# Immortal-ibr/Verifiable-Federated-Training-with-Zero-Knowledge-Proofs-ZK-FL-

Measured on AMD Instinct MI355X. Metric: Groth16 proofs/sec (training-step circuit, ~2^18 constraints) at 1/8 MI355X, higher is better.
Workload: dtype u32; 1 GPU; groth16 prove, sgd_verified(128, 4, 7, 1000) (BATCH,DIM,DEPTH,PRECISION); constraints=261399, wires=262810, domain=262144, global_batch=20, step=20 proofs per GPU (one per slot), parallelism=replicas1, slots_in_flight=20, hw_queues=28

## Files before the change

include/zkfl.h:

```cpp
#ifndef ZKFL_H
#define ZKFL_H

#include <stddef.h>
#include <stdint.h>

#ifdef __cplusplus
extern "C" {
#endif

#define ZKFL_OK 0
#define ZKFL_E_ARG -1
#define ZKFL_E_FORMAT -2
#define ZKFL_E_PRIME -3
#define ZKFL_E_MISMATCH -4
#define ZKFL_E_DEVICE -5
#define ZKFL_E_OOM -6
#define ZKFL_E_CONSTRAINT -7
#define ZKFL_E_KEY -8

typedef struct zkfl_ctx zkfl_ctx;
typedef struct zkfl_key zkfl_key;
typedef struct zkfl_witness zkfl_witness;
typedef struct zkfl_wprog zkfl_wprog;
typedef struct zkfl_vkey zkfl_vkey;
// ... 66 lines not shown
int zkfl_witness_free(zkfl_witness* w);
int zkfl_groth16_prove_resident(zkfl_ctx* ctx, zkfl_key* key, const zkfl_witness* w, const uint8_t* rs,
                                uint8_t proof_out[256]);
int zkfl_groth16_prove_batch(zkfl_ctx* ctx, zkfl_key* key, size_t n, const zkfl_witness* const* w,
                             const uint8_t* rs, uint8_t* proofs_out);

int zkfl_groth16_prove_multi(zkfl_ctx* ctx, size_t n, zkfl_key* const* keys, const zkfl_witness* const* w,
                             const uint8_t* rs, uint8_t* proofs_out);

int zkfl_zkey_load_shard(zkfl_ctx* ctx, const uint8_t* buf, size_t len, uint32_t shard, uint32_t n_shards,
                         zkfl_key** out);
int zkfl_key_shard(const zkfl_key* key, uint32_t* shard, uint32_t* n_shards);
int zkfl_groth16_prove_part_batch(zkfl_ctx* ctx, zkfl_key* key, size_t n, const zkfl_witness* const* w,
                                  const uint8_t* rs, uint8_t* parts_out);
int zkfl_groth16_assemble(zkfl_ctx* ctx, size_t n, size_t n_parts, const uint8_t* parts, const uint8_t* rs,
                          uint8_t* proofs_out);

int zkfl_debug_prove_parts(zkfl_ctx* ctx, zkfl_key* key, const uint8_t* wtns, size_t wtns_len, uint8_t* h_out,
                           uint8_t* msm_out);

int zkfl_debug_glv_split(const uint8_t k[32], uint8_t out[40]);

int zkfl_debug_g1_glv_mul(zkfl_ctx* ctx, size_t n, const uint8_t* points, const uint8_t* scalars, uint8_t* out);

int zkfl_debug_msm_front(zkfl_ctx* ctx, uint32_t n1, const size_t* n, const uint8_t* const* bases,
                         const uint8_t* const* scalars, const size_t* n_scalars, const uint32_t* const* sidx,
                         const uint32_t* extra_start, const uint8_t* const* extra, const size_t* n_extra, uint32_t b,
                         const uint8_t* bases_g2, size_t n_b, int fast, int joint, uint8_t* out_g1, uint8_t out_g2[128]);

int zkfl_debug_wtrace(zkfl_ctx* ctx, int op, uint32_t cap, void* out, uint32_t* count);

int zkfl_debug_ntt_coset(zkfl_ctx* ctx, uint8_t* data, uint32_t logn, uint32_t nvec, size_t vstride, int col_max);

int zkfl_msm_g1(zkfl_ctx* ctx, const uint8_t* bases, const uint8_t* scalars, size_t n, uint8_t out[64]);
int zkfl_msm_g2(zkfl_ctx* ctx, const uint8_t* bases, const uint8_t* scalars, size_t n, uint8_t out[128]);
int zkfl_ntt_coset(zkfl_ctx* ctx, uint8_t* data, uint32_t logn);

int zkfl_wprog_load(zkfl_ctx* ctx, const uint8_t* prog, size_t len, zkfl_wprog** out);
int zkfl_wprog_free(zkfl_wprog* prog);
int zkfl_wprog_info(const zkfl_wprog* prog, uint32_t* n_wires, uint32_t* n_inputs, uint32_t* n_public);
size_t zkfl_wtns_size(const zkfl_wprog* prog);
int zkfl_wprog_parse_inputs(const uint8_t* prog, size_t len, const char* input_json, uint8_t* inputs_out, size_t cap,
                            size_t* n_inputs);
int zkfl_witness_compute_json(zkfl_ctx* ctx, const zkfl_wprog* prog, const char* input_json, uint8_t* wtns_out);
int zkfl_witness_compute(zkfl_ctx* ctx, const zkfl_wprog* prog, size_t n, const uint8_t* inputs, uint8_t* wtns_out);
int zkfl_witness_compute_resident(zkfl_ctx* ctx, const zkfl_wprog* prog, const zkfl_key* key, size_t n,
                                  const uint8_t* inputs, zkfl_witness** out);

int zkfl_groth16_full_prove_batch(zkfl_ctx* ctx, zkfl_key* key, const zkfl_wprog* prog, size_t n,
                                  const uint8_t* inputs, const uint8_t* rs, uint8_t* proofs_out, uint8_t* pubs_out);

int zkfl_groth16_full_prove_json(zkfl_ctx* ctx, zkfl_key* key, const zkfl_wprog* prog, const char* input_json,
                                 const uint8_t* rs, uint8_t proof_out[256], uint8_t* pub_out);

int zkfl_groth16_full_prove_json_batch(zkfl_ctx* ctx, zkfl_key* key, const zkfl_wprog* prog, size_t n,
                                       const char* const* input_jsons, const uint8_t* rs, uint8_t* proofs_out,
                                       uint8_t* pubs_out);

int zkfl_groth16_full_prove_multi(zkfl_ctx* ctx, size_t n, zkfl_key* const* keys, const zkfl_wprog* const* progs,
                                  const uint8_t* const* inputs, const uint8_t* rs, uint8_t* proofs_out,
                                  uint8_t* const* pubs_out);

typedef struct zkfl_r1cs zkfl_r1cs;
typedef struct {
  uint32_t n_wires, n_pub_out, n_pub_in, n_prv_in, n_constraints;
  uint64_t n_labels, n_terms;
// ... 136 lines not shown
```

verifiable-federated-training-with-zero-knowledge-proofs-zk-fl-_amd/csrc/field.h:

```cpp
#pragma once
#include <hip/hip_runtime.h>
#include <stdint.h>

namespace zkfl {

#define ZK_DEV __device__ __forceinline__

struct FqP {
  static constexpr uint32_t P[8] = {0xd87cfd47u, 0x3c208c16u, 0x6871ca8du, 0x97816a91u,
                                    0x8181585du, 0xb85045b6u, 0xe131a029u, 0x30644e72u};
  static constexpr uint32_t ONE[8] = {0xc58f0d9du, 0xd35d438du, 0xf5c70b3du, 0x0a78eb28u,
                                      0x7879462cu, 0x666ea36fu, 0x9a07df2fu, 0x0e0a77c1u};
  static constexpr uint32_t R2[8] = {0x538afa89u, 0xf32cfc5bu, 0xd44501fbu, 0xb5e71911u,
                                     0x0a417ff6u, 0x47ab1effu, 0xcab8351fu, 0x06d89f71u};
  static constexpr uint32_t INV = 0xe4866389u;
};

struct FrP {
  static constexpr uint32_t P[8] = {0xf0000001u, 0x43e1f593u, 0x79b97091u, 0x2833e848u,
                                    0x8181585du, 0xb85045b6u, 0xe131a029u, 0x30644e72u};
  static constexpr uint32_t ONE[8] = {0x4ffffffbu, 0xac96341cu, 0x9f60cd29u, 0x36fc7695u,
                                      0x7879462eu, 0x666ea36fu, 0x9a07df2fu, 0x0e0a77c1u};
  static constexpr uint32_t R2[8] = {0xae216da7u, 0x1bb8e645u, 0xe35c59e3u, 0x53fe3ab1u,
                                     0x53bb8085u, 0x8c49833du, 0x7f4e44a5u, 0x0216d0b1u};
  static constexpr uint32_t INV = 0xefffffffu;
};

template <class PR>
struct Fp {
  uint32_t v[8];
};

using Fq = Fp<FqP>;
using Fr = Fp<FrP>;

template <class PR>
ZK_DEV Fp<PR> fp_zero() {
  Fp<PR> r;
#pragma unroll
  for (int i = 0; i < 8; i++) r.v[i] = 0;
  return r;
}

template <class PR>
ZK_DEV Fp<PR> fp_one() {
  Fp<PR> r;
#pragma unroll
  for (int i = 0; i < 8; i++) r.v[i] = PR::ONE[i];
  return r;
}

template <class PR>
ZK_DEV bool fp_is_zero(const Fp<PR>& a) {
  uint32_t x = 0;
#pragma unroll
  for (int i = 0; i < 8; i++) x |= a.v[i];
  return x == 0;
}

template <class PR>
ZK_DEV bool fp_eq(const Fp<PR>& a, const Fp<PR>& b) {
  uint32_t x = 0;
#pragma unroll
  for (int i = 0; i < 8; i++) x |= a.v[i] ^ b.v[i];
  return x == 0;
}

template <class PR>
ZK_DEV void fp_reduce_once(uint32_t r[8], const uint32_t a[8]) {
  uint32_t t[8];
  uint32_t borrow = 0;
#pragma unroll
  for (int i = 0; i < 8; i++) {
    uint64_t d = (uint64_t)a[i] - PR::P[i] - borrow;
    t[i] = (uint32_t)d;
    borrow = (uint32_t)(d >> 63);
  }
#pragma unroll
  for (int i = 0; i < 8; i++) r[i] = borrow ? a[i] : t[i];
}

template <class PR>
ZK_DEV Fp<PR> fp_add(const Fp<PR>& a, const Fp<PR>& b) {
  uint32_t s[8];
  uint64_t c = 0;
#pragma unroll
  for (int i = 0; i < 8; i++) {
    c += (uint64_t)a.v[i] + b.v[i];
    s[i] = (uint32_t)c;
    c >>= 32;
  }
  Fp<PR> r;
  fp_reduce_once<PR>(r.v, s);
  return r;
}

template <class PR>
ZK_DEV Fp<PR> fp_sub(const Fp<PR>& a, const Fp<PR>& b) {
  uint32_t d[8];
  uint32_t borrow = 0;
#pragma unroll
  for (int i = 0; i < 8; i++) {
    uint64_t t = (uint64_t)a.v[i] - b.v[i] - borrow;
    d[i] = (uint32_t)t;
    borrow = (uint32_t)(t >> 63);
  }
  uint32_t mask = 0u - borrow;
  uint64_t c = 0;
  Fp<PR> r;
#pragma unroll
  for (int i = 0; i < 8; i++) {
    c += (uint64_t)d[i] + (PR::P[i] & mask);
    r.v[i] = (uint32_t)c;
    c >>= 32;
  }
  return r;
}

template <class PR>
ZK_DEV Fp<PR> fp_neg(const Fp<PR>& a) {
  return fp_sub<PR>(fp_zero<PR>(), a);
}

template <class PR>
ZK_DEV Fp<PR> fp_dbl(const Fp<PR>& a) {
  return fp_add<PR>(a, a);
}

#define ZK_MAC_VV(lo, hi, x, y)                                                                             \
  do {                                                                                                      \
    uint64_t cc_;                                                                                           \
    asm("v_mad_u64_u32 %0, %1, %3, %4, %0\n\tv_addc_co_u32 %2, %1, %2, 0, %1" : "+v"(lo), "=&s"(cc_), "+v"(hi) \
        : "v"(x), "v"(y));                                                                                  \
  } while (0)
#define ZK_MAC_VS(lo, hi, x, y)                                                                             \
  do {                                                                                                      \
    uint64_t cc_;                                                                                           \
    asm("v_mad_u64_u32 %0, %1, %3, %4, %0\n\tv_addc_co_u32 %2, %1, %2, 0, %1" : "+v"(lo), "=&s"(cc_), "+v"(hi) \
        : "v"(x), "s"(y));                                                                                  \
  } while (0)

template <class PR>
ZK_DEV Fp<PR> fp_mul(const Fp<PR>& a, const Fp<PR>& b) {
  uint32_t m[8], u[9];
  uint64_t lo = 0;
  uint32_t hi = 0;
#pragma unroll
  for (int i = 0; i < 8; i++) {
#pragma unroll
    for (int j = 0; j < i; j++) {
      ZK_MAC_VV(lo, hi, a.v[j], b.v[i - j]);
      ZK_MAC_VS(lo, hi, m[j], PR::P[i - j]);
    }
    ZK_MAC_VV(lo, hi, a.v[i], b.v[0]);
    m[i] = (uint32_t)lo * PR::INV;
    ZK_MAC_VS(lo, hi, m[i], PR::P[0]);
    lo = (lo >> 32) | ((uint64_t)hi << 32);
    hi = 0;
  }
#pragma unroll
  for (int i = 8; i < 16; i++) {
#pragma unroll
    for (int j = i - 7; j < 8; j++) {
      ZK_MAC_VV(lo, hi, a.v[j], b.v[i - j]);
      ZK_MAC_VS(lo, hi, m[j], PR::P[i - j]);
    }
    u[i - 8] = (uint32_t)lo;
    lo = (lo >> 32) | ((uint64_t)hi << 32);
    hi = 0;
  }
  u[8] = (uint32_t)lo;
  Fp<PR> r;
  fp_reduce_once<PR>(r.v, u);
  return r;
}

template <class PR>
ZK_DEV Fp<PR> fp_mul_sum2(const Fp<PR>& a, const Fp<PR>& b, const Fp<PR>& c, const Fp<PR>& d) {
  uint32_t m[8], u[9];
  uint64_t lo = 0;
  uint32_t hi = 0;
#pragma unroll
  for (int i = 0; i < 8; i++) {
#pragma unroll
    for (int j = 0; j < i; j++) {
      ZK_MAC_VV(lo, hi, a.v[j], b.v[i - j]);
      ZK_MAC_VV(lo, hi, c.v[j], d.v[i - j]);
      ZK_MAC_VS(lo, hi, m[j], PR::P[i - j]);
    }
    ZK_MAC_VV(lo, hi, a.v[i], b.v[0]);
    ZK_MAC_VV(lo, hi, c.v[i], d.v[0]);
    m[i] = (uint32_t)lo * PR::INV;
    ZK_MAC_VS(lo, hi, m[i], PR::P[0]);
    lo = (lo >> 32) | ((uint64_t)hi << 32);
    hi = 0;
  }
#pragma unroll
  for (int i = 8; i < 16; i++) {
#pragma unroll
    for (int j = i - 7; j < 8; j++) {
      ZK_MAC_VV(lo, hi, a.v[j], b.v[i - j]);
      ZK_MAC_VV(lo, hi, c.v[j], d.v[i - j]);
      ZK_MAC_VS(lo, hi, m[j], PR::P[i - j]);
    }
    u[i - 8] = (uint32_t)lo;
    lo = (lo >> 32) | ((uint64_t)hi << 32);
    hi = 0;
  }
  u[8] = (uint32_t)lo;
  Fp<PR> r;
  fp_reduce_once<PR>(r.v, u);
  return r;
}

template <class PR>
ZK_DEV Fp<PR> fp_sqr(const Fp<PR>& a) {
  return fp_mul<PR>(a, a);
}

template <class PR>
ZK_DEV Fp<PR> fp_to_mont(const Fp<PR>& a) {
  Fp<PR> r2;
#pragma unroll
  for (int i = 0; i < 8; i++) r2.v[i] = PR::R2[i];
  return fp_mul<PR>(a, r2);
}

template <class PR>
ZK_DEV Fp<PR> fp_from_mont(const Fp<PR>& a) {
  Fp<PR> one;
  one.v[0] = 1;
#pragma unroll
  for (int i = 1; i < 8; i++) one.v[i] = 0;
  return fp_mul<PR>(a, one);
}

template <class PR>
ZK_DEV Fp<PR> fp_pow(const Fp<PR>& a, const uint32_t e[8]) {
  Fp<PR> r = fp_one<PR>();
#pragma unroll
  for (int i = 7; i >= 0; i--) {
#pragma unroll 1
    for (int b = 31; b >= 0; b--) {
      r = fp_sqr<PR>(r);
      if ((e[i] >> b) & 1u) r = fp_mul<PR>(r, a);
    }
  }
  return r;
}

template <class PR>
ZK_DEV Fp<PR> fp_inv(const Fp<PR>& a) {
  uint32_t e[8];
  uint32_t borrow = 2;
#pragma unroll
  for (int i = 0; i < 8; i++) {
    uint64_t d = (uint64_t)PR::P[i] - borrow;
    e[i] = (uint32_t)d;
    borrow = (uint32_t)(d >> 63);
  }
  return fp_pow<PR>(a, e);
}
// ... 84 lines not shown
```

verifiable-federated-training-with-zero-knowledge-proofs-zk-fl-_amd/csrc/groups.hip:

```cpp
#include <hip/hip_runtime.h>
#include <stdint.h>

#include <chrono>
#include <cstdio>
#include <vector>

#include "devbufs.h"
#include "groups.h"
#include "objects.h"

using namespace zkfl;

namespace {

ZK_DEV Fq from_m29(const Fq& a) {
  Fq c = fp_zero<FqP>();
  c.v[7] = 0x08000000u;
  return fp_mul(a, c);
}

template <class F>
ZK_DEV Affine<F> load_base(const Affine<F>* __restrict__ p) {
  Affine<F> a = *p;
  Fq* q = reinterpret_cast<Fq*>(&a);
#pragma unroll
  for (int k = 0; k < (int)(sizeof(Affine<F>) / sizeof(Fq)); k++) q[k] = from_m29(q[k]);
  return a;
}

template <class F>
__global__ void __launch_bounds__(64) k_group_sums(const Affine<F>* __restrict__ bases_w, int W, size_t n,
                                                   const uint32_t* __restrict__ start,
                                                   const uint32_t* __restrict__ members, Affine<F>* __restrict__ out) {
  const size_t j = (size_t)blockIdx.x * blockDim.x + threadIdx.x;
  if (j >= n) return;
  const Affine<F> p = load_base<F>(bases_w + j * W);
  const uint32_t b = start[j], e = start[j + 1];
  if (b == e) {
    out[j] = p;
    return;
  }
  XYZZ<F> acc = xyzz_from_affine<F>(p);
  for (uint32_t m = b; m < e; m++) acc = xyzz_madd<F>(acc, load_base<F>(bases_w + (size_t)members[m] * W));
  out[j] = xyzz_to_affine<F>(acc);
}

constexpr int DELTA_T = 256;

__global__ void __launch_bounds__(DELTA_T) k_group_delta(const Fr* __restrict__ w, const uint32_t* __restrict__ rep,
                                                         uint32_t n, Fr* __restrict__ u, uint32_t* __restrict__ cnt,
                                                         uint32_t* __restrict__ miss_out, const GroupMark M) {
  ZK_LIGHT();
  const uint32_t i = blockIdx.x * DELTA_T + threadIdx.x;
  int nz = 0;
  if (i < n) {
    const uint32_t r = rep[i];
    Fr v = fp_zero<FrP>();
    if (r != i) {
      v = fp_sub(w[i], w[r]);
#pragma unroll
      for (int k = 0; k < 8; k++) nz |= v.v[k] != 0;
    }
    u[i] = v;
  }
  if (M.wstart) {
    const unsigned long long m = __ballot(nz);
    if (m) {
      const uint32_t lane = threadIdx.x & (warpSize - 1);
      const int first = __ffsll((long long)m) - 1;
      uint32_t base = 0;
      if ((int)lane == first) base = atomicAdd(&M.state[2], (uint32_t)__popcll(m));
      base = __shfl(base, first);
      const uint32_t at = base + (uint32_t)__popcll(m & ((1ull << lane) - 1ull));
      if (nz && at < M.miss_cap) M.missing[at] = i;
    }
  }
  const int blk = __syncthreads_count(nz);
  if (threadIdx.x == 0) {
    if (blk) atomicAdd(&cnt[0], (uint32_t)blk);
    __threadfence();
    if (atomicAdd(&cnt[1], 1u) == gridDim.x - 1) {
      __threadfence();
      miss_out[0] = atomicExch(&cnt[0], 0u);
      cnt[1] = 0;
    }
  }
}

constexpr int MARK_T = 256, MARK_BLOCKS_MAX = 256;

__global__ void __launch_bounds__(MARK_T) k_group_mark(const GroupMark M) {
  ZK_LIGHT();
  const uint32_t n = M.state[2];
  if (n == 0) return;
  if (n > M.miss_cap) {
    if (blockIdx.x == 0 && threadIdx.x == 0) atomicExch(&M.state[1], 1u);
    return;
  }
  const uint32_t lane = threadIdx.x & (warpSize - 1), per = MARK_T / warpSize;
  for (uint32_t k = blockIdx.x * per + threadIdx.x / warpSize; k < n; k += gridDim.x * per) {
    if (__any((int)__atomic_load_n(&M.state[1], __ATOMIC_RELAXED))) return;
    const uint32_t i = M.missing[k], s = M.wstart[i], e = M.wstart[i + 1] & ~GROUP_ROWS_OVER;
    if (s & GROUP_ROWS_OVER) {
      if (lane == 0) atomicExch(&M.state[1], 1u);
      return;
    }
    for (uint32_t p = s + lane; p < e; p += warpSize) {
      const uint32_t j = M.wlist[p], bit = 1u << (j & 31);
      if (atomicOr(&M.state[GROUP_ROWS_STATE_BITS + (j >> 5)], bit) & bit) continue;
      const uint32_t at = atomicAdd(&M.state[0], 1u);
      if (at < M.cap) M.dirty[at] = j;
      else atomicExch(&M.state[1], 1u);
    }
  }
}

}

namespace zkfl {

template <class F>
void group_sums(hipStream_t st, const Affine<F>* bases_w, int W, size_t n, const uint32_t* start,
                const uint32_t* members, Affine<F>* out) {
  if (n) hipLaunchKernelGGL(k_group_sums<F>, dim3(zk_grid(n, 64)), dim3(64), 0, st, bases_w, W, n, start, members, out);
}
template void group_sums<FqOps>(hipStream_t, const G1Aff*, int, size_t, const uint32_t*, const uint32_t*, G1Aff*);
template void group_sums<Fq2Ops>(hipStream_t, const G2Aff*, int, size_t, const uint32_t*, const uint32_t*, G2Aff*);

void group_delta(hipStream_t st, const Fr* w, const uint32_t* rep, uint32_t n, Fr* u, uint32_t* cnt,
                 uint32_t* miss_out, const GroupMark& mark) {
  hipLaunchKernelGGL(k_group_delta, dim3(zk_grid(n, DELTA_T)), dim3(DELTA_T), 0, st, w, rep, n, u, cnt, miss_out, mark);
}

void group_mark_rows(hipStream_t st, const GroupMark& mark) {
  const unsigned blocks = std::min<unsigned>(zk_grid((size_t)mark.miss_cap * 64, MARK_T), MARK_BLOCKS_MAX);
  hipLaunchKernelGGL(k_group_mark, dim3(blocks), dim3(MARK_T), 0, st, mark);
}

void key_groups_release(zkfl_key* k) {
  msm_bases_free(k->gA);
  msm_bases_free(k->gB1);
  msm_bases_free(k->gB2);
  msm_bases_free(k->gCH);
  void* ptrs[] = {k->grp.d_rep,    k->grp.d_cls,    k->grp.d_crp,  k->grp.d_cterms,
                  k->grp.d_ccoefs, k->grp.d_wstart, k->grp.d_wlist};
  for (void* p : ptrs)
    if (p) (void)hipFree(p);
  const uint32_t builds = k->grp.builds;
  k->grp = KeyGroups();
  k->grp.builds = builds;
}

}

namespace {

template <class F>
hipError_t build_query(const MsmBases<F>& plain, MsmBases<F>& out, const GroupQuery& q, uint32_t extra_start,
                       DevBufs& D, hipStream_t st) {
  ZK_CHECK(msm_bases_alloc(out, plain.n, plain.c));
  if (plain.n == 0) return hipSuccess;
  uint32_t *d_start, *d_members;
  Affine<F>* d_img;
  ZK_CHECK(D.get(&d_start, q.start.size()));
// ... 259 lines not shown
```

verifiable-federated-training-with-zero-knowledge-proofs-zk-fl-_amd/csrc/ntt.hip:

```cpp
#include "ntt.h"
#include "devbufs.h"
#include "fr_consts.h"
#include "wtrace.h"

namespace zkfl {

#ifndef NTT_LDS_LOG_BITS
#define NTT_LDS_LOG_BITS 10
#endif
constexpr int NTT_LDS_LOG = NTT_LDS_LOG_BITS;
constexpr int NTT_LDS_N = 1 << NTT_LDS_LOG;

__global__ void k_ntt_twiddles(Fr* __restrict__ tw, size_t half, Fr root_mont) {
  size_t i = (size_t)blockIdx.x * blockDim.x + threadIdx.x;
  if (i >= half) return;
  Fr acc = fp_one<FrP>();
  Fr base = root_mont;
  size_t e = i;
  while (e) {
    if (e & 1) acc = fp_mul(acc, base);
    base = fp_sqr(base);
    e >>= 1;
  }
  tw[i] = acc;
// ... 18 lines not shown
                                size_t twstride, int nvec, size_t vstride) {
  size_t t = (size_t)blockIdx.x * blockDim.x + threadIdx.x;
  size_t nb = n >> 1;
  if (t >= nb * nvec) return;
  size_t v = t / nb;
  t -= v * nb;
  Fr* x = a + v * vstride;
  size_t j = t & (half - 1);
  size_t i0 = ((t - j) << 1) + j;
  size_t i1 = i0 + half;
  Fr u = x[i0], w = x[i1];
  x[i0] = fp_add(u, w);
  x[i1] = fp_mul(fp_sub(u, w), tw[j * twstride]);
}

__global__ void k_ntt_dit_stage(Fr* __restrict__ a, size_t n, size_t half, const Fr* __restrict__ tw,
                                size_t twstride, int nvec, size_t vstride) {
  size_t t = (size_t)blockIdx.x * blockDim.x + threadIdx.x;
  size_t nb = n >> 1;
  if (t >= nb * nvec) return;
  size_t v = t / nb;
  t -= v * nb;
  Fr* x = a + v * vstride;
  size_t j = t & (half - 1);
  size_t i0 = ((t - j) << 1) + j;
  size_t i1 = i0 + half;
  Fr u = x[i0];
  Fr w = fp_mul(x[i1], tw[j * twstride]);
  x[i0] = fp_add(u, w);
  x[i1] = fp_sub(u, w);
}

template <bool DIF>
__global__ void __launch_bounds__(512) k_ntt_lds(Fr* __restrict__ a, size_t n, int logt,
                                                 const Fr* __restrict__ tw, int nvec, size_t vstride,
                                                 const Fr* __restrict__ scale) {
  __shared__ Fr tile[NTT_LDS_N];
  const size_t T = (size_t)1 << logt;
  const size_t tiles_per_vec = n >> logt;
  const size_t tile_id = blockIdx.x;
  const size_t v = tile_id / tiles_per_vec;
  if (v >= (size_t)nvec) return;
  Fr* x = a + v * vstride + (tile_id - v * tiles_per_vec) * T;
  for (size_t i = threadIdx.x; i < T; i += blockDim.x) tile[i] = x[i];
  __syncthreads();
  const size_t nbf = T >> 1;
  for (int s = 0; s < logt; s++) {
    const size_t half = DIF ? (T >> (s + 1)) : ((size_t)1 << s);
    const size_t len = half << 1;
    const size_t twstride = n / len;
    for (size_t t = threadIdx.x; t < nbf; t += blockDim.x) {
      size_t j = t & (half - 1);
      size_t i0 = ((t - j) << 1) + j;
      size_t i1 = i0 + half;
      Fr u = tile[i0], w = tile[i1];
      Fr tws = tw[j * twstride];
      if (DIF) {
        tile[i0] = fp_add(u, w);
        tile[i1] = fp_mul(fp_sub(u, w), tws);
      } else {
        w = fp_mul(w, tws);
        tile[i0] = fp_add(u, w);
        tile[i1] = fp_sub(u, w);
      }
    }
    __syncthreads();
  }
  const size_t base = (tile_id - v * tiles_per_vec) * T;
  if (scale)
    for (size_t i = threadIdx.x; i < T; i += blockDim.x) x[i] = fp_mul(tile[i], scale[base + i]);
  else
    for (size_t i = threadIdx.x; i < T; i += blockDim.x) x[i] = tile[i];
}

__global__ void __launch_bounds__(512) k_ntt_lds_pair(Fr* __restrict__ a, size_t n, int logt,
                                                      const Fr* __restrict__ tw_inv, const Fr* __restrict__ tw_fwd,
                                                      int nvec, size_t vstride, const Fr* __restrict__ scale) {
  ZK_WT(WT_NTT_LDS);
  ZK_LIGHT();
  __shared__ Fr tile[NTT_LDS_N];
  const size_t T = (size_t)1 << logt;
  const size_t tiles_per_vec = n >> logt;
  const size_t tile_id = blockIdx.x;
  const size_t v = tile_id / tiles_per_vec;
  if (v >= (size_t)nvec) return;
  const size_t base = (tile_id - v * tiles_per_vec) * T;
  Fr* x = a + v * vstride + base;
  for (size_t i = threadIdx.x; i < T; i += blockDim.x) tile[i] = x[i];
  __syncthreads();
  const size_t nbf = T >> 1;
  for (int s = 0; s < logt; s++) {
    const size_t half = T >> (s + 1), twstride = n / (half << 1);
    for (size_t t = threadIdx.x; t < nbf; t += blockDim.x) {
      const size_t j = t & (half - 1), i0 = ((t - j) << 1) + j, i1 = i0 + half;
      const Fr u = tile[i0], w = tile[i1];
      tile[i0] = fp_add(u, w);
      tile[i1] = fp_mul(fp_sub(u, w), tw_inv[j * twstride]);
    }
    __syncthreads();
  }
  for (size_t i = threadIdx.x; i < T; i += blockDim.x) tile[i] = fp_mul(tile[i], scale[base + i]);
  __syncthreads();
  for (int s = 0; s < logt; s++) {
    const size_t half = (size_t)1 << s, twstride = n / (half << 1);
    for (size_t t = threadIdx.x; t < nbf; t += blockDim.x) {
      const size_t j = t & (half - 1), i0 = ((t - j) << 1) + j, i1 = i0 + half;
      const Fr u = tile[i0], w = fp_mul(tile[i1], tw_fwd[j * twstride]);
      tile[i0] = fp_add(u, w);
      tile[i1] = fp_sub(u, w);
    }
    __syncthreads();
  }
  for (size_t i = threadIdx.x; i < T; i += blockDim.x) x[i] = tile[i];
}

template <bool DIF>
__global__ void __launch_bounds__(256) k_ntt_lds4(Fr* __restrict__ a, size_t n, int logt, const Fr* __restrict__ tw,
                                                  int nvec, size_t vstride, const Fr* __restrict__ scale) {
  __shared__ Fr tile[NTT_LDS_N];
  const uint32_t T = 1u << logt;
  const size_t tiles_per_vec = n >> logt;
  const size_t tile_id = blockIdx.x;
  const size_t v = tile_id / tiles_per_vec;
  if (v >= (size_t)nvec) return;
  Fr* x = a + v * vstride + (tile_id - v * tiles_per_vec) * T;
  for (uint32_t i = threadIdx.x; i < T; i += blockDim.x) tile[i] = x[i];
  __syncthreads();
  const uint32_t t = threadIdx.x;
  int s = 0;
  for (; s + 1 < logt; s += 2) {
    if (t < (T >> 2)) {
      if (DIF) {
        const uint32_t h2 = T >> (s + 2), h1 = h2 << 1;
        const uint32_t j = t & (h2 - 1), i0 = ((t - j) << 2) + j;
        const size_t st1 = n / (2 * (size_t)h1), st2 = 2 * st1;
        const Fr xa = tile[i0], xb = tile[i0 + h2], xc = tile[i0 + h1], xd = tile[i0 + h1 + h2];
        const Fr a1 = fp_add(xa, xc), c1 = fp_mul(fp_sub(xa, xc), tw[j * st1]);
        const Fr b1 = fp_add(xb, xd), d1 = fp_mul(fp_sub(xb, xd), tw[(j + h2) * st1]);
        const Fr w2 = tw[j * st2];
        tile[i0] = fp_add(a1, b1);
        tile[i0 + h2] = fp_mul(fp_sub(a1, b1), w2);
        tile[i0 + h1] = fp_add(c1, d1);
        tile[i0 + h1 + h2] = fp_mul(fp_sub(c1, d1), w2);
// ... 228 lines not shown
```

verifiable-federated-training-with-zero-knowledge-proofs-zk-fl-_amd/csrc/zkfl.hip:

```cpp
#include <hip/hip_runtime.h>
#include <stdint.h>
#include <string.h>
#include <sys/random.h>

#include <algorithm>
#include <cstdlib>
#include <string>
#include <type_traits>
#include <vector>

#include "assemble.h"
#include "devbufs.h"
#include "glv.h"
#include "host_parse.h"
#include "merkle.h"
#include "objects.h"
#include "poly.h"
#include "setup.h"
#include "verify.h"
#include "witness.h"

using namespace zkfl;

static thread_local std::string g_err;
// ... 328 lines not shown
  return run_msm_primitive<Fq2Ops>(ctx, bases, scalars, n, out);
}

int zkfl_debug_ntt_coset(zkfl_ctx* ctx, uint8_t* data, uint32_t logn, uint32_t nvec, size_t vstride, int col_max) {
  if (!ctx || !data || logn < 1 || logn > 27 || nvec < 1 || nvec > 3 || col_max > NTT_COL_TILE_LOG)
    return fail(ZKFL_E_ARG, "ntt: bad args");
  const size_t n = (size_t)1 << logn;
  if (vstride < n || vstride > ((size_t)1 << 32)) return fail(ZKFL_E_ARG, "ntt: bad stride");
  hipStream_t st = ctx->st;
  struct Plan {
    NttPlan pl;
    ~Plan() { ntt_plan_free(pl); }
  } P;
  DevBufs D;
  Fr* d;
  const size_t count = (size_t)(nvec - 1) * vstride + n;
  HIP_TRY(ntt_plan_alloc(P.pl, (int)logn, st), "ntt");
  if (col_max >= 0) P.pl.col_max = col_max;
  HIP_TRY(D.get(&d, count), "ntt");
  HIP_TRY(hipMemcpyAsync(d, data, count * 32, hipMemcpyHostToDevice, st), "ntt");
  for (uint32_t v = 0; v < nvec; v++) fr_std_to_mont(st, d + v * vstride, n);
  HIP_TRY(ntt_coset_shift(P.pl, d, (int)nvec, vstride, st), "ntt");
  for (uint32_t v = 0; v < nvec; v++) fr_mont_to_std(st, d + v * vstride, n);
  HIP_TRY(hipGetLastError(), "ntt");
  HIP_TRY(hipMemcpyAsync(data, d, count * 32, hipMemcpyDeviceToHost, st), "ntt");
  HIP_TRY(hipStreamSynchronize(st), "ntt");
  return ZKFL_OK;
}

int zkfl_ntt_coset(zkfl_ctx* ctx, uint8_t* data, uint32_t logn) {
  return zkfl_debug_ntt_coset(ctx, data, logn, 1, logn <= 27 ? (size_t)1 << logn : 0, -1);
}

static int setup_gen_mul_abi(zkfl_ctx* ctx, const uint8_t* scalars, size_t n, uint8_t* out, bool g2) {
  if (!ctx || !scalars || !out) return fail(ZKFL_E_ARG, "gen_mul: bad args");
  hipError_t e = setup_gen_mul(g2, ctx->st, scalars, n, out);
  return e == hipSuccess ? ZKFL_OK : hip_fail(e, "gen_mul");
}

int zkfl_setup_g1_gen_mul(zkfl_ctx* ctx, const uint8_t* scalars, size_t n, uint8_t* out) {
  return setup_gen_mul_abi(ctx, scalars, n, out, false);
}

int zkfl_setup_g2_gen_mul(zkfl_ctx* ctx, const uint8_t* scalars, size_t n, uint8_t* out) {
  return setup_gen_mul_abi(ctx, scalars, n, out, true);
}

static int setup_scale_abi(zkfl_ctx* ctx, const uint8_t* points, const uint8_t* scalars, size_t n, uint8_t* out,
                           bool g2) {
  if (!ctx || (n && (!points || !scalars || !out))) return fail(ZKFL_E_ARG, "setup scale: bad args");
  hipError_t e = setup_scale(g2, ctx->st, points, scalars, n, out);
  return e == hipSuccess ? ZKFL_OK : hip_fail(e, "setup scale");
}

int zkfl_setup_g1_scale(zkfl_ctx* ctx, const uint8_t* points, const uint8_t* scalars, size_t n, uint8_t* out) {
  return setup_scale_abi(ctx, points, scalars, n, out, false);
}

int zkfl_setup_g2_scale(zkfl_ctx* ctx, const uint8_t* points, const uint8_t* scalars, size_t n, uint8_t* out) {
  return setup_scale_abi(ctx, points, scalars, n, out, true);
}

static int setup_lagrange_abi(zkfl_ctx* ctx, const uint8_t* points, uint32_t logn, uint8_t* out, bool g2) {
  if (!ctx || !points || !out) return fail(ZKFL_E_ARG, "setup lagrange: bad args");
  if (logn > 28) return fail(ZKFL_E_ARG, "setup lagrange: logn > 28 (BN254 Fr 2-adicity)");
  hipError_t e = setup_lagrange(g2, ctx->st, points, (int)logn, out);
// ... 532 lines not shown
```

verifiable-federated-training-with-zero-knowledge-proofs-zk-fl-_amd/zkfl/native.py:

```python

from __future__ import annotations

import ctypes as C
import os

_PKG_DIR = os.path.dirname(os.path.dirname(os.path.abspath(__file__)))
LIB_PATH = os.path.abspath(os.environ["ZKFL_LIB"]) if os.environ.get("ZKFL_LIB") else os.path.join(_PKG_DIR, "libzkfl.so")

ZKFL_OK = 0
PART_BYTES = 768
PART_LAYOUT = {"A": (0, 128), "B1": (128, 256), "B2": (256, 512), "C": (512, 640), "H": (640, 768)}
ERRORS = {
    -1: "ZKFL_E_ARG", -2: "ZKFL_E_FORMAT", -3: "ZKFL_E_PRIME", -4: "ZKFL_E_MISMATCH",
    -5: "ZKFL_E_DEVICE", -6: "ZKFL_E_OOM", -7: "ZKFL_E_CONSTRAINT", -8: "ZKFL_E_KEY",
}

_P = C.c_void_p
_U8P = C.POINTER(C.c_uint8)


class R1csHeader(C.Structure):
    _fields_ = [("n_wires", C.c_uint32), ("n_pub_out", C.c_uint32), ("n_pub_in", C.c_uint32),
                ("n_prv_in", C.c_uint32), ("n_constraints", C.c_uint32), ("n_labels", C.c_uint64),
                ("n_terms", C.c_uint64)]
# ... 85 lines not shown
    "zkfl_debug_ab_partition": (C.c_int, [C.c_char_p, C.c_char_p, C.c_size_t, C.c_uint32, C.c_uint32,
                                          C.POINTER(C.c_uint32), C.POINTER(C.c_uint32), _U8P]),
    "zkfl_key_set_groups": (C.c_int, [_P, C.POINTER(C.c_uint32), C.c_size_t]),
    "zkfl_key_learn_groups": (C.c_int, [_P, _P, _P]),
    "zkfl_key_groups": (C.c_int, [_P, C.POINTER(GroupsInfo)]),
    "zkfl_key_group_rows": (C.c_int, [_P, C.POINTER(GroupRowsInfo)]),
    "zkfl_debug_groups": (C.c_int, [C.c_char_p, C.c_char_p, C.c_size_t, C.POINTER(C.c_uint32), C.POINTER(C.c_uint32),
                                    C.c_size_t, C.c_uint32, C.POINTER(C.c_uint32), C.POINTER(C.c_uint32),
                                    C.POINTER(C.c_uint32)]),
    "zkfl_debug_group_rows": (C.c_int, [C.POINTER(C.c_uint32), C.c_uint32, C.POINTER(C.c_uint32), C.c_uint32,
                                        C.POINTER(C.c_uint32), C.POINTER(C.c_uint32), C.c_uint32, C.c_uint32,
                                        C.c_uint32] + [C.POINTER(C.c_uint32)] * 7),
    "zkfl_debug_abc": (C.c_int, [_P, _P, _P, C.c_int, _U8P, C.POINTER(C.c_uint32)]),
    "zkfl_key_set_slots": (C.c_int, [_P, C.c_int]),
    "zkfl_groth16_prove": (C.c_int, [_P, _P, C.c_char_p, C.c_size_t, C.c_char_p, _U8P, _U8P,
                                     C.POINTER(C.c_size_t)]),
    "zkfl_witness_upload": (C.c_int, [_P, _P, C.c_char_p, C.c_size_t, C.POINTER(_P)]),
    "zkfl_witness_free": (C.c_int, [_P]),
    "zkfl_groth16_prove_resident": (C.c_int, [_P, _P, _P, C.c_char_p, _U8P]),
    "zkfl_groth16_prove_batch": (C.c_int, [_P, _P, C.c_size_t, C.POINTER(_P), C.c_char_p, _U8P]),
    "zkfl_debug_prove_parts": (C.c_int, [_P, _P, C.c_char_p, C.c_size_t, _U8P, _U8P]),
    "zkfl_debug_glv_split": (C.c_int, [C.c_char_p, _U8P]),
    "zkfl_debug_g1_glv_mul": (C.c_int, [_P, C.c_size_t, C.c_char_p, C.c_char_p, _U8P]),
    "zkfl_debug_msm_front": (C.c_int, [_P, C.c_uint32, C.POINTER(C.c_size_t), C.POINTER(C.c_char_p),
                                       C.POINTER(C.c_char_p), C.POINTER(C.c_size_t),
                                       C.POINTER(C.POINTER(C.c_uint32)), C.POINTER(C.c_uint32), C.POINTER(C.c_char_p),
                                       C.POINTER(C.c_size_t), C.c_uint32, C.c_char_p, C.c_size_t, C.c_int, C.c_int,
                                       _U8P, _U8P]),
    "zkfl_debug_wtrace": (C.c_int, [_P, C.c_int, C.c_uint32, _P, C.POINTER(C.c_uint32)]),
    "zkfl_msm_g1": (C.c_int, [_P, C.c_char_p, C.c_char_p, C.c_size_t, _U8P]),
    "zkfl_msm_g2": (C.c_int, [_P, C.c_char_p, C.c_char_p, C.c_size_t, _U8P]),
    "zkfl_ntt_coset": (C.c_int, [_P, _U8P, C.c_uint32]),
    "zkfl_debug_ntt_coset": (C.c_int, [_P, _U8P, C.c_uint32, C.c_uint32, C.c_size_t, C.c_int]),
    "zkfl_setup_g1_gen_mul": (C.c_int, [_P, C.c_char_p, C.c_size_t, _U8P]),
    "zkfl_setup_g2_gen_mul": (C.c_int, [_P, C.c_char_p, C.c_size_t, _U8P]),
    "zkfl_setup_g1_scale": (C.c_int, [_P, C.c_char_p, C.c_char_p, C.c_size_t, _U8P]),
    "zkfl_setup_g2_scale": (C.c_int, [_P, C.c_char_p, C.c_char_p, C.c_size_t, _U8P]),
    "zkfl_setup_g1_lagrange": (C.c_int, [_P, C.c_char_p, C.c_uint32, _U8P]),
    "zkfl_setup_g2_lagrange": (C.c_int, [_P, C.c_char_p, C.c_uint32, _U8P]),
    "zkfl_setup_g1_lincomb": (C.c_int, [_P, C.c_char_p, C.c_size_t, C.c_size_t, C.POINTER(C.c_uint64),
                                        C.POINTER(C.c_uint32), C.c_char_p, _U8P]),
    "zkfl_setup_g2_lincomb": (C.c_int, [_P, C.c_char_p, C.c_size_t, C.c_size_t, C.POINTER(C.c_uint64),
                                        C.POINTER(C.c_uint32), C.c_char_p, _U8P]),
    "zkfl_groth16_verify": (C.c_int, [_P, C.c_char_p, C.c_size_t, C.c_char_p, C.c_size_t, C.c_char_p]),
    "zkfl_groth16_verify_batch": (C.c_int, [_P, C.c_char_p, C.c_size_t, C.c_size_t, C.c_char_p, C.c_size_t,
                                            C.c_char_p, C.POINTER(C.c_int32)]),
    "zkfl_pairing": (C.c_int, [_P, C.c_size_t, C.c_char_p, C.c_char_p, _U8P]),
    "zkfl_debug_miller_loop": (C.c_int, [_P, C.c_size_t, C.c_char_p, C.c_char_p, _U8P]),
    "zkfl_vkey_load": (C.c_int, [_P, C.c_char_p, C.c_size_t, C.POINTER(_P)]),
    "zkfl_vkey_info": (C.c_int, [_P, C.POINTER(C.c_uint32)]),
    "zkfl_vkey_free": (C.c_int, [_P]),
    "zkfl_groth16_verify_multi": (C.c_int, [_P, C.c_size_t, C.POINTER(_P), C.POINTER(C.c_char_p),
                                            C.POINTER(C.c_size_t), C.c_char_p, C.POINTER(C.c_int32), C.c_int]),
    "zkfl_groth16_verify_round": (C.c_int, [_P, C.c_size_t, C.POINTER(_P), C.POINTER(C.c_char_p),
                                            C.POINTER(C.c_size_t), C.c_char_p, C.c_char_p, C.POINTER(C.c_int32),
                                            C.POINTER(C.c_uint32)]),
    "zkfl_debug_verify_round": (C.c_int, [_P, C.c_size_t, C.POINTER(_P), C.POINTER(C.c_char_p),
                                          C.POINTER(C.c_size_t), C.c_char_p, C.c_char_p, C.c_size_t, _U8P,
                                          C.POINTER(C.c_int32)]),
    "zkfl_debug_wave_pairing": (C.c_int,[_P, C.c_size_t, C.c_char_p, C.c_char_p, C.c_int, _U8P]),
    "zkfl_wprog_load": (C.c_int, [_P, C.c_char_p, C.c_size_t, C.POINTER(_P)]),
    "zkfl_wprog_free": (C.c_int, [_P]),
    "zkfl_wprog_info": (C.c_int, [_P, C.POINTER(C.c_uint32), C.POINTER(C.c_uint32), C.POINTER(C.c_uint32)]),
    "zkfl_wtns_size": (C.c_size_t, [_P]),
    "zkfl_witness_compute": (C.c_int, [_P, _P, C.c_size_t, C.c_char_p, _U8P]),
    "zkfl_witness_compute_resident": (C.c_int, [_P, _P, _P, C.c_size_t, C.c_char_p, C.POINTER(_P)]),
# ... 249 lines not shown
            self.h, n1, arr(C.c_size_t, [len(s[0]) // 64 for s in full]), arr(C.c_char_p, [s[0] for s in full]),
            arr(C.c_char_p, [s[1] for s in full]), arr(C.c_size_t, [len(s[1]) // 32 for s in full]),
            arr(C.POINTER(C.c_uint32), [C.cast(m, C.POINTER(C.c_uint32)) if m is not None else None for m in maps]),
            arr(C.c_uint32, [s[3] for s in full]), arr(C.c_char_p, [s[4] for s in full]),
            arr(C.c_size_t, [len(s[4]) // 32 for s in full]), b, bases_g2, len(bases_g2) // 128, int(fast),
            int(joint), out1, out2))
        o = bytes(out1)
        return [o[64 * i:64 * i + 64] for i in range(n1)], bytes(out2)

    def msm_g2(self, bases: bytes, scalars: bytes) -> bytes:
        n = len(scalars) // 32
        assert len(bases) == 128 * n
        out = _buf(128)
        check(lib().zkfl_msm_g2(self.h, bases, scalars, n, out))
        return bytes(out)

    def ntt_coset(self, data: bytes) -> bytes:
        n = len(data) // 32
        logn = n.bit_length() - 1
        assert 1 << logn == n
        buf = (C.c_uint8 * len(data)).from_buffer_copy(data)
        check(lib().zkfl_ntt_coset(self.h, buf, logn))
        return bytes(buf)

    def debug_ntt_coset(self, data: bytes, logn: int, nvec: int = 1, vstride: int | None = None,
                        col_max: int = -1) -> bytes:
        n = 1 << logn
        vstride = n if vstride is None else vstride
        assert len(data) == ((nvec - 1) * vstride + n) * 32
        buf = (C.c_uint8 * len(data)).from_buffer_copy(data)
        check(lib().zkfl_debug_ntt_coset(self.h, buf, logn, nvec, vstride, col_max))
        return bytes(buf)

    def g1_gen_mul(self, scalars: bytes) -> bytes:
        n = len(scalars) // 32
        out = _buf(64 * n if n else 1)
        check(lib().zkfl_setup_g1_gen_mul(self.h, scalars, n, out))
        return bytes(out)[:64 * n]

    def g2_gen_mul(self, scalars: bytes) -> bytes:
        n = len(scalars) // 32
        out = _buf(128 * n if n else 1)
        check(lib().zkfl_setup_g2_gen_mul(self.h, scalars, n, out))
        return bytes(out)[:128 * n]

    def _scale(self, fn, size, points: bytes, scalars: bytes) -> bytes:
        n = len(scalars) // 32
        if len(points) != size * n or len(scalars) != 32 * n:
            raise ZkflError(-1, f"scale: {len(points)} B of points for {n} scalars")
        out = _buf(size * n if n else 1)
        check(fn(self.h, points, scalars, n, out))
        return bytes(out)[:size * n]

    def g1_scale(self, points: bytes, scalars: bytes) -> bytes:
        return self._scale(lib().zkfl_setup_g1_scale, 64, points, scalars)

    def g2_scale(self, points: bytes, scalars: bytes) -> bytes:
        return self._scale(lib().zkfl_setup_g2_scale, 128, points, scalars)

    def _lagrange(self, fn, size, points: bytes, logn: int) -> bytes:
        if len(points) != size << logn:
            raise ZkflError(-1, f"lagrange: expected {1 << logn} points")
        out = _buf(size << logn)
        check(fn(self.h, points, logn, out))
        return bytes(out)

# ... 573 lines not shown
```

Measured before the change: 856.4 proofs/s.

## Fuse first/last NTT LDS stages with loads/scale and cap group-delta grid

The LDS NTT kernels now fuse the trivial first (DIT) or last (DIF) radix-2 stage with the global load or the scaled store. Twiddle-free j==0 butterflies in the half==2 stage skip the multiply, and the pair kernel folds the coset scale into the adjacent butterflies. This cuts LDS round-trips, barriers and some multiplies. The group-delta kernel becomes grid-stride with at most 512 blocks and reduces counts per wave, which lowers the per-block atomic traffic. Field helpers become host-callable and a debug coset-join entry point is added for testing.

```diff
diff --git a/include/zkfl.h b/include/zkfl.h
--- a/include/zkfl.h
+++ b/include/zkfl.h
@@ -122,6 +122,8 @@
 
 int zkfl_debug_ntt_coset(zkfl_ctx* ctx, uint8_t* data, uint32_t logn, uint32_t nvec, size_t vstride, int col_max);
 
+int zkfl_debug_coset_join(zkfl_ctx* ctx, const uint8_t* abc, uint32_t logn, int col_max, uint8_t* h_out);
+
 int zkfl_msm_g1(zkfl_ctx* ctx, const uint8_t* bases, const uint8_t* scalars, size_t n, uint8_t out[64]);
 int zkfl_msm_g2(zkfl_ctx* ctx, const uint8_t* bases, const uint8_t* scalars, size_t n, uint8_t out[128]);
 int zkfl_ntt_coset(zkfl_ctx* ctx, uint8_t* data, uint32_t logn);
diff --git a/verifiable-federated-training-with-zero-knowledge-proofs-zk-fl-_amd/csrc/field.h b/verifiable-federated-training-with-zero-knowledge-proofs-zk-fl-_amd/csrc/field.h
--- a/verifiable-federated-training-with-zero-knowledge-proofs-zk-fl-_amd/csrc/field.h
+++ b/verifiable-federated-training-with-zero-knowledge-proofs-zk-fl-_amd/csrc/field.h
@@ -5,6 +5,7 @@
 namespace zkfl {
 
 #define ZK_DEV __device__ __forceinline__
+#define ZK_HD __host__ __device__ __forceinline__
 
 struct FqP {
   static constexpr uint32_t P[8] = {0xd87cfd47u, 0x3c208c16u, 0x6871ca8du, 0x97816a91u,
@@ -35,7 +36,7 @@
 using Fr = Fp<FrP>;
 
 template <class PR>
-ZK_DEV Fp<PR> fp_zero() {
+ZK_HD Fp<PR> fp_zero() {
   Fp<PR> r;
 #pragma unroll
   for (int i = 0; i < 8; i++) r.v[i] = 0;
@@ -43,7 +44,7 @@
 }
 
 template <class PR>
-ZK_DEV Fp<PR> fp_one() {
+ZK_HD Fp<PR> fp_one() {
   Fp<PR> r;
 #pragma unroll
   for (int i = 0; i < 8; i++) r.v[i] = PR::ONE[i];
@@ -51,7 +52,7 @@
 }
 
 template <class PR>
-ZK_DEV bool fp_is_zero(const Fp<PR>& a) {
+ZK_HD bool fp_is_zero(const Fp<PR>& a) {
   uint32_t x = 0;
 #pragma unroll
   for (int i = 0; i < 8; i++) x |= a.v[i];
@@ -59,7 +60,7 @@
 }
 
 template <class PR>
-ZK_DEV bool fp_eq(const Fp<PR>& a, const Fp<PR>& b) {
+ZK_HD bool fp_eq(const Fp<PR>& a, const Fp<PR>& b) {
   uint32_t x = 0;
 #pragma unroll
   for (int i = 0; i < 8; i++) x |= a.v[i] ^ b.v[i];
@@ -67,7 +68,7 @@
 }
 
 template <class PR>
-ZK_DEV void fp_reduce_once(uint32_t r[8], const uint32_t a[8]) {
+ZK_HD void fp_reduce_once(uint32_t r[8], const uint32_t a[8]) {
   uint32_t t[8];
   uint32_t borrow = 0;
 #pragma unroll
@@ -81,7 +82,7 @@
 }
 
 template <class PR>
-ZK_DEV Fp<PR> fp_add(const Fp<PR>& a, const Fp<PR>& b) {
+ZK_HD Fp<PR> fp_add(const Fp<PR>& a, const Fp<PR>& b) {
   uint32_t s[8];
   uint64_t c = 0;
 #pragma unroll
@@ -96,7 +97,7 @@
 }
 
 template <class PR>
-ZK_DEV Fp<PR> fp_sub(const Fp<PR>& a, const Fp<PR>& b) {
+ZK_HD Fp<PR> fp_sub(const Fp<PR>& a, const Fp<PR>& b) {
   uint32_t d[8];
   uint32_t borrow = 0;
 #pragma unroll
@@ -118,15 +119,16 @@
 }
 
 template <class PR>
-ZK_DEV Fp<PR> fp_neg(const Fp<PR>& a) {
+ZK_HD Fp<PR> fp_neg(const Fp<PR>& a) {
   return fp_sub<PR>(fp_zero<PR>(), a);
 }
 
 template <class PR>
-ZK_DEV Fp<PR> fp_dbl(const Fp<PR>& a) {
+ZK_HD Fp<PR> fp_dbl(const Fp<PR>& a) {
   return fp_add<PR>(a, a);
 }
 
+#if defined(__HIP_DEVICE_COMPILE__)
 #define ZK_MAC_VV(lo, hi, x, y)                                                                             \
   do {                                                                                                      \
     uint64_t cc_;                                                                                           \
@@ -139,9 +141,18 @@
     asm("v_mad_u64_u32 %0, %1, %3, %4, %0\n\tv_addc_co_u32 %2, %1, %2, 0, %1" : "+v"(lo), "=&s"(cc_), "+v"(hi) \
         : "v"(x), "s"(y));                                                                                  \
   } while (0)
-
-template <class PR>
-ZK_DEV Fp<PR> fp_mul(const Fp<PR>& a, const Fp<PR>& b) {
+#else
+#define ZK_MAC_VV(lo, hi, x, y)                       \
+  do {                                                \
+    const uint64_t p_ = (uint64_t)(x) * (uint64_t)(y); \
+    lo += p_;                                         \
+    hi += lo < p_;                                    \
+  } while (0)
+#define ZK_MAC_VS(lo, hi, x, y) ZK_MAC_VV(lo, hi, x, y)
+#endif
+
+template <class PR>
+ZK_HD Fp<PR> fp_mul(const Fp<PR>& a, const Fp<PR>& b) {
   uint32_t m[8], u[9];
   uint64_t lo = 0;
   uint32_t hi = 0;
@@ -176,7 +187,7 @@
 }
 
 template <class PR>
-ZK_DEV Fp<PR> fp_mul_sum2(const Fp<PR>& a, const Fp<PR>& b, const Fp<PR>& c, const Fp<PR>& d) {
+ZK_HD Fp<PR> fp_mul_sum2(const Fp<PR>& a, const Fp<PR>& b, const Fp<PR>& c, const Fp<PR>& d) {
   uint32_t m[8], u[9];
   uint64_t lo = 0;
   uint32_t hi = 0;
@@ -214,12 +225,12 @@
 }
 
 template <class PR>
-ZK_DEV Fp<PR> fp_sqr(const Fp<PR>& a) {
+ZK_HD Fp<PR> fp_sqr(const Fp<PR>& a) {
   return fp_mul<PR>(a, a);
 }
 
 template <class PR>
-ZK_DEV Fp<PR> fp_to_mont(const Fp<PR>& a) {
+ZK_HD Fp<PR> fp_to_mont(const Fp<PR>& a) {
   Fp<PR> r2;
 #pragma unroll
   for (int i = 0; i < 8; i++) r2.v[i] = PR::R2[i];
@@ -227,7 +238,7 @@
 }
 
 template <class PR>
-ZK_DEV Fp<PR> fp_from_mont(const Fp<PR>& a) {
+ZK_HD Fp<PR> fp_from_mont(const Fp<PR>& a) {
   Fp<PR> one;
   one.v[0] = 1;
 #pragma unroll
diff --git a/verifiable-federated-training-with-zero-knowledge-proofs-zk-fl-_amd/csrc/groups.hip b/verifiable-federated-training-with-zero-knowledge-proofs-zk-fl-_amd/csrc/groups.hip
--- a/verifiable-federated-training-with-zero-knowledge-proofs-zk-fl-_amd/csrc/groups.hip
+++ b/verifiable-federated-training-with-zero-knowledge-proofs-zk-fl-_amd/csrc/groups.hip
@@ -45,27 +45,28 @@
   out[j] = xyzz_to_affine<F>(acc);
 }
 
-constexpr int DELTA_T = 256;
+constexpr int DELTA_T = 256, DELTA_BLOCKS_MAX = 512;
 
 __global__ void __launch_bounds__(DELTA_T) k_group_delta(const Fr* __restrict__ w, const uint32_t* __restrict__ rep,
                                                          uint32_t n, Fr* __restrict__ u, uint32_t* __restrict__ cnt,
                                                          uint32_t* __restrict__ miss_out, const GroupMark M) {
   ZK_LIGHT();
-  const uint32_t i = blockIdx.x * DELTA_T + threadIdx.x;
-  int nz = 0;
-  if (i < n) {
-    const uint32_t r = rep[i];
-    Fr v = fp_zero<FrP>();
-    if (r != i) {
-      v = fp_sub(w[i], w[r]);
+  int blk = 0;
+  for (uint32_t b0 = blockIdx.x * DELTA_T; b0 < n; b0 += gridDim.x * DELTA_T) {
+    const uint32_t i = b0 + threadIdx.x;
+    int nz = 0;
+    if (i < n) {
+      const uint32_t r = rep[i];
+      Fr v = fp_zero<FrP>();
+      if (r != i) {
+        v = fp_sub(w[i], w[r]);
 #pragma unroll
-      for (int k = 0; k < 8; k++) nz |= v.v[k] != 0;
-    }
-    u[i] = v;
-  }
-  if (M.wstart) {
+        for (int k = 0; k < 8; k++) nz |= v.v[k] != 0;
+      }
+      u[i] = v;
+    }
     const unsigned long long m = __ballot(nz);
-    if (m) {
+    if (m && M.wstart) {
       const uint32_t lane = threadIdx.x & (warpSize - 1);
       const int first = __ffsll((long long)m) - 1;
       uint32_t base = 0;
@@ -74,9 +75,15 @@
       const uint32_t at = base + (uint32_t)__popcll(m & ((1ull << lane) - 1ull));
       if (nz && at < M.miss_cap) M.missing[at] = i;
     }
-  }
-  const int blk = __syncthreads_count(nz);
+    blk += nz;
+  }
+  __shared__ int wave_nz[DELTA_T / 64];
+  for (int off = warpSize / 2; off; off >>= 1) blk += __shfl_xor(blk, off);
+  if ((threadIdx.x & (warpSize - 1)) == 0) wave_nz[threadIdx.x / warpSize] = blk;
+  __syncthreads();
   if (threadIdx.x == 0) {
+    blk = 0;
+    for (int k = 0; k < DELTA_T / warpSize; k++) blk += wave_nz[k];
     if (blk) atomicAdd(&cnt[0], (uint32_t)blk);
     __threadfence();
     if (atomicAdd(&cnt[1], 1u) == gridDim.x - 1) {
@@ -129,7 +136,8 @@
 
 void group_delta(hipStream_t st, const Fr* w, const uint32_t* rep, uint32_t n, Fr* u, uint32_t* cnt,
                  uint32_t* miss_out, const GroupMark& mark) {
-  hipLaunchKernelGGL(k_group_delta, dim3(zk_grid(n, DELTA_T)), dim3(DELTA_T), 0, st, w, rep, n, u, cnt, miss_out, mark);
+  const unsigned blocks = std::min<unsigned>(zk_grid(n, DELTA_T), DELTA_BLOCKS_MAX);
+  hipLaunchKernelGGL(k_group_delta, dim3(blocks), dim3(DELTA_T), 0, st, w, rep, n, u, cnt, miss_out, mark);
 }
 
 void group_mark_rows(hipStream_t st, const GroupMark& mark) {
diff --git a/verifiable-federated-training-with-zero-knowledge-proofs-zk-fl-_amd/csrc/ntt.hip b/verifiable-federated-training-with-zero-knowledge-proofs-zk-fl-_amd/csrc/ntt.hip
--- a/verifiable-federated-training-with-zero-knowledge-proofs-zk-fl-_amd/csrc/ntt.hip
+++ b/verifiable-federated-training-with-zero-knowledge-proofs-zk-fl-_amd/csrc/ntt.hip
@@ -74,6 +74,28 @@
 }
 
 template <bool DIF>
+ZK_DEV void ntt_lds_stage(Fr* tile, size_t nbf, size_t half, const Fr* __restrict__ tw, size_t twstride) {
+  const size_t hb = nbf >> 1;
+  for (size_t t = threadIdx.x; t < nbf; t += blockDim.x) {
+    const size_t q = half == 2 ? (t < hb ? t << 1 : ((t - hb) << 1) | 1) : t;
+    const size_t j = q & (half - 1), i0 = ((q - j) << 1) + j, i1 = i0 + half;
+    const Fr u = tile[i0];
+    Fr w = tile[i1];
+    if (half == 2 && j == 0) {
+      tile[i0] = fp_add(u, w);
+      tile[i1] = fp_sub(u, w);
+    } else if (DIF) {
+      tile[i0] = fp_add(u, w);
+      tile[i1] = fp_mul(fp_sub(u, w), tw[j * twstride]);
+    } else {
+      w = fp_mul(w, tw[j * twstride]);
+      tile[i0] = fp_add(u, w);
+      tile[i1] = fp_sub(u, w);
+    }
+  }
+}
+
+template <bool DIF>
 __global__ void __launch_bounds__(512) k_ntt_lds(Fr* __restrict__ a, size_t n, int logt,
                                                  const Fr* __restrict__ tw, int nvec, size_t vstride,
                                                  const Fr* __restrict__ scale) {
@@ -83,36 +105,39 @@
   const size_t tile_id = blockIdx.x;
   const size_t v = tile_id / tiles_per_vec;
   if (v >= (size_t)nvec) return;
-  Fr* x = a + v * vstride + (tile_id - v * tiles_per_vec) * T;
-  for (size_t i = threadIdx.x; i < T; i += blockDim.x) tile[i] = x[i];
-  __syncthreads();
+  const size_t base = (tile_id - v * tiles_per_vec) * T;
+  Fr* x = a + v * vstride + base;
   const size_t nbf = T >> 1;
-  for (int s = 0; s < logt; s++) {
-    const size_t half = DIF ? (T >> (s + 1)) : ((size_t)1 << s);
-    const size_t len = half << 1;
-    const size_t twstride = n / len;
+  if (DIF) {
+    for (size_t i = threadIdx.x; i < T; i += blockDim.x) tile[i] = x[i];
+    __syncthreads();
+    for (int s = 0; s + 1 < logt; s++) {
+      ntt_lds_stage<true>(tile, nbf, T >> (s + 1), tw, n / (T >> s));
+      __syncthreads();
+    }
     for (size_t t = threadIdx.x; t < nbf; t += blockDim.x) {
-      size_t j = t & (half - 1);
-      size_t i0 = ((t - j) << 1) + j;
-      size_t i1 = i0 + half;
-      Fr u = tile[i0], w = tile[i1];
-      Fr tws = tw[j * twstride];
-      if (DIF) {
-        tile[i0] = fp_add(u, w);
-        tile[i1] = fp_mul(fp_sub(u, w), tws);
-      } else {
-        w = fp_mul(w, tws);
-        tile[i0] = fp_add(u, w);
-        tile[i1] = fp_sub(u, w);
+      const Fr u = tile[2 * t], w = tile[2 * t + 1];
+      Fr r0 = fp_add(u, w), r1 = fp_sub(u, w);
+      if (scale) {
+        r0 = fp_mul(r0, scale[base + 2 * t]);
+        r1 = fp_mul(r1, scale[base + 2 * t + 1]);
       }
-    }
-    __syncthreads();
-  }
-  const size_t base = (tile_id - v * tiles_per_vec) * T;
-  if (scale)
-    for (size_t i = threadIdx.x; i < T; i += blockDim.x) x[i] = fp_mul(tile[i], scale[base + i]);
-  else
+      x[2 * t] = r0;
+      x[2 * t + 1] = r1;
+    }
+  } else {
+    for (size_t t = threadIdx.x; t < nbf; t += blockDim.x) {
+      const Fr u = x[2 * t], w = x[2 * t + 1];
+      tile[2 * t] = fp_add(u, w);
+      tile[2 * t + 1] = fp_sub(u, w);
+    }
+    __syncthreads();
+    for (int s = 1; s < logt; s++) {
+      ntt_lds_stage<false>(tile, nbf, (size_t)1 << s, tw, n / ((size_t)2 << s));
+      __syncthreads();
+    }
     for (size_t i = threadIdx.x; i < T; i += blockDim.x) x[i] = tile[i];
+  }
 }
 
 __global__ void __launch_bounds__(512) k_ntt_lds_pair(Fr* __restrict__ a, size_t n, int logt,
@@ -131,26 +156,19 @@
   for (size_t i = threadIdx.x; i < T; i += blockDim.x) tile[i] = x[i];
   __syncthreads();
   const size_t nbf = T >> 1;
-  for (int s = 0; s < logt; s++) {
-    const size_t half = T >> (s + 1), twstride = n / (half << 1);
-    for (size_t t = threadIdx.x; t < nbf; t += blockDim.x) {
-      const size_t j = t & (half - 1), i0 = ((t - j) << 1) + j, i1 = i0 + half;
-      const Fr u = tile[i0], w = tile[i1];
-      tile[i0] = fp_add(u, w);
-      tile[i1] = fp_mul(fp_sub(u, w), tw_inv[j * twstride]);
-    }
-    __syncthreads();
-  }
-  for (size_t i = threadIdx.x; i < T; i += blockDim.x) tile[i] = fp_mul(tile[i], scale[base + i]);
+  for (int s = 0; s + 1 < logt; s++) {
+    ntt_lds_stage<true>(tile, nbf, T >> (s + 1), tw_inv, n / (T >> s));
+    __syncthreads();
+  }
+  for (size_t t = threadIdx.x; t < nbf; t += blockDim.x) {
+    const Fr u = tile[2 * t], w = tile[2 * t + 1];
+    const Fr y0 = fp_mul(fp_add(u, w), scale[base + 2 * t]), y1 = fp_mul(fp_sub(u, w), scale[base + 2 * t + 1]);
+    tile[2 * t] = fp_add(y0, y1);
+    tile[2 * t + 1] = fp_sub(y0, y1);
+  }
   __syncthreads();
-  for (int s = 0; s < logt; s++) {
-    const size_t half = (size_t)1 << s, twstride = n / (half << 1);
-    for (size_t t = threadIdx.x; t < nbf; t += blockDim.x) {
-      const size_t j = t & (half - 1), i0 = ((t - j) << 1) + j, i1 = i0 + half;
-      const Fr u = tile[i0], w = fp_mul(tile[i1], tw_fwd[j * twstride]);
-      tile[i0] = fp_add(u, w);
-      tile[i1] = fp_sub(u, w);
-    }
+  for (int s = 1; s < logt; s++) {
+    ntt_lds_stage<false>(tile, nbf, (size_t)1 << s, tw_fwd, n / ((size_t)2 << s));
     __syncthreads();
   }
   for (size_t i = threadIdx.x; i < T; i += blockDim.x) x[i] = tile[i];
diff --git a/verifiable-federated-training-with-zero-knowledge-proofs-zk-fl-_amd/csrc/zkfl.hip b/verifiable-federated-training-with-zero-knowledge-proofs-zk-fl-_amd/csrc/zkfl.hip
--- a/verifiable-federated-training-with-zero-knowledge-proofs-zk-fl-_amd/csrc/zkfl.hip
+++ b/verifiable-federated-training-with-zero-knowledge-proofs-zk-fl-_amd/csrc/zkfl.hip
@@ -384,6 +384,31 @@
   return zkfl_debug_ntt_coset(ctx, data, logn, 1, logn <= 27 ? (size_t)1 << logn : 0, -1);
 }
 
+int zkfl_debug_coset_join(zkfl_ctx* ctx, const uint8_t* abc, uint32_t logn, int col_max, uint8_t* h_out) {
+  if (!ctx || !abc || !h_out || logn < 1 || logn > 27 || col_max > NTT_COL_TILE_LOG)
+    return fail(ZKFL_E_ARG, "coset join: bad args");
+  const size_t n = (size_t)1 << logn;
+  hipStream_t st = ctx->st;
+  struct Plan {
+    NttPlan pl;
+    ~Plan() { ntt_plan_free(pl); }
+  } P;
+  DevBufs D;
+  Fr *d, *h;
+  HIP_TRY(ntt_plan_alloc(P.pl, (int)logn, st), "coset join");
+  if (col_max >= 0) P.pl.col_max = col_max;
+  HIP_TRY(D.get(&d, 3 * n), "coset join");
+  HIP_TRY(D.get(&h, n), "coset join");
+  HIP_TRY(hipMemcpyAsync(d, abc, 3 * n * 32, hipMemcpyHostToDevice, st), "coset join");
+  fr_std_to_mont(st, d, 3 * n);
+  HIP_TRY(ntt_coset_shift(P.pl, d, 3, n, st), "coset join");
+  join_h(st, d, n, h);
+  HIP_TRY(hipGetLastError(), "coset join");
+  HIP_TRY(hipMemcpyAsync(h_out, h, n * 32, hipMemcpyDeviceToHost, st), "coset join");
+  HIP_TRY(hipStreamSynchronize(st), "coset join");
+  return ZKFL_OK;
+}
+
 static int setup_gen_mul_abi(zkfl_ctx* ctx, const uint8_t* scalars, size_t n, uint8_t* out, bool g2) {
   if (!ctx || !scalars || !out) return fail(ZKFL_E_ARG, "gen_mul: bad args");
   hipError_t e = setup_gen_mul(g2, ctx->st, scalars, n, out);
diff --git a/verifiable-federated-training-with-zero-knowledge-proofs-zk-fl-_amd/zkfl/native.py b/verifiable-federated-training-with-zero-knowledge-proofs-zk-fl-_amd/zkfl/native.py
--- a/verifiable-federated-training-with-zero-knowledge-proofs-zk-fl-_amd/zkfl/native.py
+++ b/verifiable-federated-training-with-zero-knowledge-proofs-zk-fl-_amd/zkfl/native.py
@@ -141,6 +141,7 @@
     "zkfl_msm_g2": (C.c_int, [_P, C.c_char_p, C.c_char_p, C.c_size_t, _U8P]),
     "zkfl_ntt_coset": (C.c_int, [_P, _U8P, C.c_uint32]),
     "zkfl_debug_ntt_coset": (C.c_int, [_P, _U8P, C.c_uint32, C.c_uint32, C.c_size_t, C.c_int]),
+    "zkfl_debug_coset_join": (C.c_int, [_P, C.c_char_p, C.c_uint32, C.c_int, _U8P]),
     "zkfl_setup_g1_gen_mul": (C.c_int, [_P, C.c_char_p, C.c_size_t, _U8P]),
     "zkfl_setup_g2_gen_mul": (C.c_int, [_P, C.c_char_p, C.c_size_t, _U8P]),
     "zkfl_setup_g1_scale": (C.c_int, [_P, C.c_char_p, C.c_char_p, C.c_size_t, _U8P]),
@@ -456,6 +457,13 @@
         check(lib().zkfl_debug_ntt_coset(self.h, buf, logn, nvec, vstride, col_max))
         return bytes(buf)
 
+    def debug_coset_join(self, abc: bytes, logn: int, col_max: int = -1) -> bytes:
+        n = 1 << logn
+        assert len(abc) == 3 * n * 32
+        out = _buf(32 * n)
+        check(lib().zkfl_debug_coset_join(self.h, abc, logn, col_max, out))
+        return bytes(out)
+
     def g1_gen_mul(self, scalars: bytes) -> bytes:
         n = len(scalars) // 32
         out = _buf(64 * n if n else 1)
```

Result: faster. 883.1 proofs/s (median of 6 runs) (+3.1%).
